# vtuber-plan/vcvits

Hardware: AMD Instinct MI355X
Metric: training utterances/sec (gen+disc step) at base.json segment_size (higher is better)
Workload: dtype f32; 1 GPU; configs/base.json widths, HiFi-GAN generator + MPD(8 periods+S) + MSD + STFT/mel-L1, G step + D step + AdamW (learning rate 0: weights held at their seeded initial values); per_gpu_batch=16, global_batch=16, segment_size=16384, parallelism=dp1, process_group_ranks=1, graph_recording_steps_before_warmup=3

## Files before the change

### include/vcvits_hip.h

```cpp
#ifndef VCVITS_HIP_H
#define VCVITS_HIP_H

#include <stdint.h>

#ifdef __cplusplus
extern "C" {
#endif

#define VCV_OK 0
#define VCV_EINVAL (-1)
#define VCV_EHIP (-2)
#define VCV_ELDS (-3)

#define VCV_ACT_NONE 0
#define VCV_ACT_LEAKY 1
#define VCV_ACT_RELU 2
#define VCV_ACT_TANH 3
#define VCV_ACT_LOGCLAMP 4

#define VCV_TF_NONE 0
#define VCV_TF_LEAKY 1
#define VCV_TF_DLEAKY 2
#define VCV_TF_DRELU 3
#define VCV_TF_DTANH 4
// ... 100 lines not shown

int vcv_conv_m1_fwd(const float* x, const float* w, const float* bias, float* y, int B, int C, int Tin,
                    int Tout, int P, int K, int stride, int dil, int pad, int in_leaky, int out_act,
                    float slope, void* stream);
int vcv_conv_c1_fwd(const float* x, const float* w, const float* bias, float* y, int B, int M, int Tin, int Tout,
                    int P, int K, int stride, int dil, int pad, int out_act, float slope, void* stream);
int vcv_conv_c1_fwd_masked(const float* x, const float* w, const float* bias, float* y, const float* oaux, int B, int M,
                           int Tin, int Tout, int P, int K, int stride, int dil, int pad, int out_act, float slope,
                           void* stream);
int vcv_conv_c1_fwd_flip(const float* x, const float* w, const float* bias, float* y, const float* oaux, int B, int M, int Tin,
                         int Tout, int P, int K, int stride, int dil, int pad, int out_act, float slope, int flip_taps,
                         void* stream);
int vcv_conv_c1_dgrad(const float* dy, const float* w, float* dx, int B, int M, int Tin, int Tout, int P, int K,
                      int stride, int dil, int pad, void* stream);
int vcv_linear_t1_fwd(const float* x, const float* w, const float* bias, float* y, int B, int C, int M, void* stream);
int vcv_linear_t1_dgrad(const float* dy, const float* w, float* dx, int B, int C, int M, void* stream);
int vcv_linear_t1_wgrad(const float* dy, const float* x, float* dw, int B, int C, int M, void* stream);
int vcv_thin_wgrad(const float* a, const float* bsh, const float* aaux, const float* baux, float* dw, int B,
                   int M, int C, int Ta, int Tb, int P, int K, int s, int d, int off, int a_tf, int b_tf,
                   float slope, float alpha, void* stream);

int vcv_grouped41_fwd(const float* x, const float* w, const float* bias, float* y, int B, int G, int Mg, int Tin,
                      int Tout, int out_act, float slope, void* stream);
int vcv_grouped41_fwd_bf16(const float* x, const float* w, const float* bias, float* y, int B, int G, int Mg, int Tin, int Tout,
                           int out_act, float slope, void* stream);
int vcv_grouped41_dgrad(const float* dy, const float* yaux, const float* w, float* dx, int B, int G, int Mg, int Tin,
                        int Tout, int dtf, float slope, void* stream);
int vcv_grouped41_dgrad_bf16(const float* dy, const float* yaux, const float* w, float* dx, int B, int G, int Mg, int Tin, int Tout,
                             int dtf, float slope, void* stream);
int vcv_grouped41_wgrad(const float* dy, const float* yaux, const float* x, float* dw, int B, int G, int Mg, int Tin,
                        int Tout, int dtf, float slope, void* stream);
int vcv_grouped41_wgrad_bf16(const float* dy, const float* yaux, const float* x, float* dw, int B, int G, int Mg, int Tin, int Tout,
                             int dtf, float slope, void* stream);

int vcv_bias_grad(const float* dy, const float* aux, float* dbias, int B, int C, int T, int tf, float slope,
                  int accumulate, void* stream);

int vcv_weight_norm_fwd(const float* v, const float* g, float* w, float* norm, int R, int C, void* stream);
int vcv_weight_norm_bwd(const float* dw, const float* v, const float* g, const float* norm, float* dv,
                        float* dg, int R, int C, void* stream);
int vcv_weight_norm_many_fwd(const void* items_dev, int n_items, int total_rows, float* wbuf, float* norm,
                             void* stream);
int vcv_weight_norm_many_bwd(const void* items_dev, int n_items, int total_rows, const float* norm, void* stream);

int vcv_spectral_norm_fwd(const float* w, float* u, float* v, float* w_sn, float* sigma, float* work, int R, int N,
                          int power_iteration, float eps, void* stream);
int vcv_spectral_norm_bwd(const float* dw_sn, const float* w_sn, const float* u, const float* v, const float* sigma,
                          float* dw, float* work, int R, int N, void* stream);

int vcv_weight_flip_transpose(const float* w, float* wt, int M, int C, int K, void* stream);

int vcv_act_grad(const float* dy, const float* y, float* out, int tf, float slope, int64_t n, void* stream);
int vcv_act_grad_add(const float* dy, const float* add, const float* y, float* out, int tf, float slope, int64_t n, void* stream);
int vcv_act_grad_bias(const float* dy, const float* y, float* out, float* dbias, int B, int C, int T, int tf, float slope,
                      void* stream);

int vcv_avg3(const float* a, const float* b, const float* c, float* y, int64_t n, void* stream);
int vcv_scale(const float* x, float* y, float alpha, int64_t n, void* stream);
int vcv_mask_mul(const float* x, const float* mask, float* y, int B, int C, int T, void* stream);
int vcv_reflect_pad_fwd(const float* x, float* y, int R, int T, int Tp, void* stream);
int vcv_reflect_pad_bwd(const float* dy, float* dx, int R, int T, int Tp, void* stream);
int vcv_avgpool4_fwd(const float* x, float* y, int R, int T, void* stream);
int vcv_avgpool4_bwd(const float* dy, float* dx, int R, int T, void* stream);

int vcv_loss_sum(const float* a, const float* b, float target, int mode, float scale, float* out,
                 int64_t n, void* stream);
// ... 186 lines not shown
```

### vcvits_amd/_lib.py

```python
import ctypes
import os

import torch

_HERE = os.path.dirname(os.path.abspath(__file__))
from . import tuning

LIB_PATH = tuning.text("VCVITS_HIP_LIB", "", "path of another build of libvcvits_hip.so (A/B builds)") or \
    os.path.join(_HERE, "csrc", "libvcvits_hip.so")

VCV_OK = 0
ACT_NONE, ACT_LEAKY, ACT_RELU, ACT_TANH, ACT_LOGCLAMP = 0, 1, 2, 3, 4
TF_NONE, TF_LEAKY, TF_DLEAKY, TF_DRELU, TF_DTANH, TF_DLOGCLAMP = 0, 1, 2, 3, 4, 5

_f32p = ctypes.c_void_p
_i32 = ctypes.c_int32


class VcvConvArgs(ctypes.Structure):
    _fields_ = [
        ("x", _f32p), ("w", _f32p), ("bias", _f32p), ("res", _f32p), ("mask", _f32p),
        ("xaux", _f32p), ("oaux", _f32p), ("y", _f32p),
        ("B", _i32), ("G", _i32), ("Cg", _i32), ("Mg", _i32),
        ("Tin", _i32), ("Tout", _i32), ("P", _i32),
# ... 39 lines not shown
_lib = None


def lib():
    global _lib
    if _lib is None:
        if not os.path.exists(LIB_PATH):
            raise RuntimeError(
                "libvcvits_hip.so not found at %s -- run `python -m vcvits_amd.build_ext` "
                "(there is no CPU fallback for the vcvits hot path)" % LIB_PATH)
        L = ctypes.CDLL(LIB_PATH)
        L.vcv_version.restype = ctypes.c_char_p
        for name in EXPORTS:
            fn = getattr(L, name)
            if name != "vcv_version":
                fn.restype = (ctypes.c_int64 if name in ("vcv_conv_dma_workspace", "vcv_wgrad_bf16_scratch", "vcv_wgrad_x3_scratch", "vcv_layernorm_c_bwd_scratch", "vcv_resblock_pair_supported",
                                                                "vcv_rel_attn_stream_bwd_workspace")
                              else ctypes.c_void_p if name == "vcv_get_seed_offset_ptr" else ctypes.c_int)
                fn.argtypes = _ARGTYPES[name]
        _lib = L
    return _lib


EXPORTS = [
    "vcv_version", "vcv_conv_gemm", "vcv_conv_wgrad", "vcv_conv_wgrad_takes_dma", "vcv_conv_wgrad_split_terms", "vcv_bias_grad",
    "vcv_weight_norm_fwd", "vcv_weight_norm_bwd", "vcv_spectral_norm_fwd", "vcv_spectral_norm_bwd", "vcv_avg3", "vcv_scale", "vcv_mask_mul",
    "vcv_reflect_pad_fwd", "vcv_reflect_pad_bwd", "vcv_avgpool4_fwd", "vcv_avgpool4_bwd",
    "vcv_loss_sum", "vcv_loss_grad", "vcv_adamw", "vcv_stft_mag_fwd", "vcv_stft_mag_bwd",
    "vcv_wn_gate_fwd", "vcv_wn_gate_bwd", "vcv_row_sum", "vcv_wn_res_skip_fwd", "vcv_wn_res_skip_bwd",
    "vcv_split_sample_fwd", "vcv_split_sample_bwd", "vcv_coupling", "vcv_layernorm_c_fwd",
    "vcv_layernorm_c_bwd", "vcv_rel_softmax_fwd", "vcv_rel_value_fwd", "vcv_rel_softmax_bwd",
    "vcv_kl_fwd", "vcv_kl_bwd", "vcv_nearest_fwd", "vcv_nearest_bwd", "vcv_nearest_raw_fwd", "vcv_nearest_raw_bwd", "vcv_slice_fwd", "vcv_slice_bwd",
    "vcv_dropout", "vcv_prof_begin", "vcv_prof_end", "vcv_prof_dump", "vcv_conv_m1_fwd", "vcv_conv_c1_fwd", "vcv_conv_c1_fwd_masked", "vcv_conv_c1_fwd_flip", "vcv_conv_c1_dgrad", "vcv_linear_t1_fwd", "vcv_linear_t1_dgrad", "vcv_linear_t1_wgrad", "vcv_thin_wgrad", "vcv_weight_flip_transpose",
    "vcv_act_grad", "vcv_act_grad_add", "vcv_weight_norm_many_fwd", "vcv_weight_norm_many_bwd", "vcv_loss_many_sum", "vcv_loss_many_grad", "vcv_conv_dma_workspace", "vcv_conv_dma", "vcv_conv_dma_plan", "vcv_conv_dma_run", "vcv_stft_complex_fwd", "vcv_istft", "vcv_grouped41_fwd", "vcv_grouped41_fwd_bf16", "vcv_grouped41_dgrad", "vcv_grouped41_dgrad_bf16", "vcv_grouped41_wgrad", "vcv_grouped41_wgrad_bf16",
    "vcv_prior_sample", "vcv_prof_bytes", "vcv_conv_bf16_plan", "vcv_conv_bf16_run", "vcv_wgrad_bf16_scratch", "vcv_wgrad_bf16", "vcv_act_grad_bias", "vcv_conv_pk_plan", "vcv_conv_pk_run",
    "vcv_conv_x3_plan", "vcv_conv_x3_run", "vcv_conv_x3_set_terms", "vcv_conv_x3_get_terms", "vcv_conv_x3_set_all", "vcv_wgrad_x3_scratch", "vcv_wgrad_x3", "vcv_rel_attn_supported", "vcv_rel_attn_fwd", "vcv_rel_attn_bwd", "vcv_rel_attn_bwd2", "vcv_set_deterministic", "vcv_get_deterministic", "vcv_prof_roof", "vcv_prof_pause", "vcv_conv_x3_pack_job", "vcv_conv_pk_pack_job", "vcv_conv_bf16_pack_job", "vcv_pack_many", "vcv_upload_table",
    "vcv_conv_bf16io_plan", "vcv_conv_bf16io_run", "vcv_cast_f32_x16", "vcv_cast_x16_f32", "vcv_conv_m1_x16_fwd",
    "vcv_prof_active", "vcv_set_seed_offset_ptr", "vcv_get_seed_offset_ptr", "vcv_pack_many_prepared", "vcv_adamw_dev", "vcv_set_words", "vcv_tuning_set", "vcv_tuning_get", "vcv_embedding_t_fwd", "vcv_embedding_t_fwd_checked", "vcv_embedding_t_bwd", "vcv_conv_x3_set_variant", "vcv_conv_plan_describe", "vcv_wgrad_bf16_set_force", "vcv_layernorm_c_bwd_scratch", "vcv_layernorm_c_bwd_ws", "vcv_resblock_pair_supported", "vcv_resblock_pair_pack", "vcv_resblock_pair_x16",
    "vcv_pyin_yin", "vcv_pyin_obs", "vcv_pyin_viterbi",
    "vcv_resample_table", "vcv_resample_apply", "vcv_phase_vocoder", "vcv_istft_ordered",
    "vcv_hubert_bias_gelu", "vcv_hubert_groupnorm_gelu", "vcv_hubert_layernorm_c_gelu", "vcv_hubert_attn_supported", "vcv_hubert_attn_fwd",
    "vcv_hubert_groupnorm_gelu_len", "vcv_hubert_mask_frames", "vcv_hubert_attn_fwd_len",
    "vcv_rel_attn_stream_supported", "vcv_rel_attn_stream_fwd",
    "vcv_rel_attn_stream_train_fwd", "vcv_rel_attn_stream_bwd_workspace", "vcv_rel_attn_stream_bwd",
    "vcv_rel_attn_stream_fwd_bf16", "vcv_hubert_attn_fwd_bf16", "vcv_hubert_attn_fwd_len_bf16",
]


_P, _I, _L, _F, _D = ctypes.c_void_p, ctypes.c_int, ctypes.c_int64, ctypes.c_float, ctypes.c_double
_ARGTYPES = {
    "vcv_conv_gemm": [ctypes.POINTER(VcvConvArgs), _P],
    "vcv_conv_wgrad": [ctypes.POINTER(VcvWgradArgs), _P],
    "vcv_conv_wgrad_takes_dma": [ctypes.POINTER(VcvWgradArgs)],
    "vcv_conv_wgrad_split_terms": [ctypes.POINTER(VcvWgradArgs)],
    "vcv_bias_grad": [_P, _P, _P, _I, _I, _I, _I, _F, _I, _P],
    "vcv_weight_norm_fwd": [_P, _P, _P, _P, _I, _I, _P],
    "vcv_weight_norm_bwd": [_P, _P, _P, _P, _P, _P, _I, _I, _P],
    "vcv_spectral_norm_fwd": [_P, _P, _P, _P, _P, _P, _I, _I, _I, _F, _P],
    "vcv_spectral_norm_bwd": [_P, _P, _P, _P, _P, _P, _P, _I, _I, _P],
    "vcv_avg3": [_P, _P, _P, _P, _L, _P],
    "vcv_scale": [_P, _P, _F, _L, _P],
    "vcv_mask_mul": [_P, _P, _P, _I, _I, _I, _P],
    "vcv_reflect_pad_fwd": [_P, _P, _I, _I, _I, _P],
    "vcv_reflect_pad_bwd": [_P, _P, _I, _I, _I, _P],
    "vcv_avgpool4_fwd": [_P, _P, _I, _I, _P],
    "vcv_avgpool4_bwd": [_P, _P, _I, _I, _P],
    "vcv_loss_sum": [_P, _P, _F, _I, _F, _P, _L, _P],
# ... 20 lines not shown
    "vcv_dropout": [_P, _P, _L, _F, ctypes.c_uint64, _P],
    "vcv_rel_value_fwd": [_P, _P, _P, _I, _I, _I, _I, _I, _P],
    "vcv_rel_softmax_bwd": [_P, _P, _P, _P, _P, _P, _P, _P, _P, _P, _P, _P, _I, _I, _I, _I, _I, _F, _P],
    "vcv_rel_attn_supported": [_I, _I, _I, _I, _I],
    "vcv_rel_attn_fwd": [_P, _P, _P, _P, _P, _P, _P, _P, _P, _I, _I, _I, _I, _I, _F, _F, ctypes.c_uint64, _I, _P],
    "vcv_rel_attn_bwd": [_P, _P, _P, _P, _P, _P, _P, _P, _P, _P, _P, _P, _P, _P, _I, _I, _I, _I, _I, _F, _F, ctypes.c_uint64, _I, _P],
    "vcv_rel_attn_bwd2": [_P, _P, _P, _P, _P, _P, _P, _P, _P, _P, _P, _P, _P, _P, _P, _I, _I, _I, _I, _I, _F, _F, ctypes.c_uint64, _I, _P],
    "vcv_set_deterministic": [_I],
    "vcv_get_deterministic": [],
    "vcv_kl_fwd": [_P, _P, _P, _P, _P, _P, _I, _I, _I, _P],
    "vcv_kl_bwd": [_P, _P, _P, _P, _P, _P, _P, _P, _P, _P, _I, _I, _I, _P],
    "vcv_nearest_fwd": [_P, _P, _I, _I, _I, _P],
    "vcv_nearest_bwd": [_P, _P, _I, _I, _I, _P],
    "vcv_nearest_raw_fwd": [_P, _P, _I, _I, _I, _P, _P],
    "vcv_nearest_raw_bwd": [_P, _P, _I, _I, _I, _P, _P],
    "vcv_slice_fwd": [_P, _P, _I, _P, _I, _I, _I, _I, _P],
    "vcv_slice_bwd": [_P, _P, _I, _P, _I, _I, _I, _I, _P],
    "vcv_conv_m1_fwd": [_P, _P, _P, _P, _I, _I, _I, _I, _I, _I, _I, _I, _I, _I, _I, _F, _P],
    "vcv_conv_c1_fwd": [_P, _P, _P, _P, _I, _I, _I, _I, _I, _I, _I, _I, _I, _I, _F, _P],
    "vcv_conv_c1_fwd_masked": [_P, _P, _P, _P, _P, _I, _I, _I, _I, _I, _I, _I, _I, _I, _I, _F, _P],
    "vcv_conv_c1_fwd_flip": [_P, _P, _P, _P, _P, _I, _I, _I, _I, _I, _I, _I, _I, _I, _I, _F, _I, _P],
    "vcv_linear_t1_fwd": [_P, _P, _P, _P, _I, _I, _I, _P],
    "vcv_linear_t1_dgrad": [_P, _P, _P, _I, _I, _I, _P],
    "vcv_linear_t1_wgrad": [_P, _P, _P, _I, _I, _I, _P],
    "vcv_conv_c1_dgrad": [_P, _P, _P, _I, _I, _I, _I, _I, _I, _I, _I, _I, _P],
    "vcv_thin_wgrad": [_P, _P, _P, _P, _P, _I, _I, _I, _I, _I, _I, _I, _I, _I, _I, _I, _I, _F, _F, _P],
    "vcv_weight_flip_transpose": [_P, _P, _I, _I, _I, _P],
    "vcv_grouped41_fwd": [_P, _P, _P, _P, _I, _I, _I, _I, _I, _I, _F, _P],
    "vcv_grouped41_fwd_bf16": [_P, _P, _P, _P, _I, _I, _I, _I, _I, _I, _F, _P],
    "vcv_grouped41_dgrad": [_P, _P, _P, _P, _I, _I, _I, _I, _I, _I, _F, _P],
    "vcv_grouped41_dgrad_bf16": [_P, _P, _P, _P, _I, _I, _I, _I, _I, _I, _F, _P],
    "vcv_grouped41_wgrad": [_P, _P, _P, _P, _I, _I, _I, _I, _I, _I, _F, _P],
    "vcv_grouped41_wgrad_bf16": [_P, _P, _P, _P, _I, _I, _I, _I, _I, _I, _F, _P],
    "vcv_act_grad": [_P, _P, _P, _I, _F, _L, _P],
    "vcv_act_grad_add": [_P, _P, _P, _P, _I, _F, _L, _P],
    "vcv_act_grad_bias": [_P, _P, _P, _P, _I, _I, _I, _I, _F, _P],
    "vcv_stft_complex_fwd": [_P, _P, _P, _P, _I, _I, _I, _I, _I, _I, _P],
    "vcv_istft": [_P, _P, _P, _P, _P, _I, _I, _I, _I, _I, _P],
    "vcv_loss_many_sum": [_P, _I, _I, _F, _I, _P, _P],
    "vcv_loss_many_grad": [_P, _I, _I, _F, _I, _P, _P, _P],
    "vcv_weight_norm_many_fwd": [_P, _I, _I, _P, _P, _P],
    "vcv_weight_norm_many_bwd": [_P, _I, _I, _P, _P],
    "vcv_conv_dma_workspace": [ctypes.POINTER(VcvConvArgs)],
    "vcv_conv_dma": [ctypes.POINTER(VcvConvArgs), _P, _I, _P],
    "vcv_conv_dma_plan": [ctypes.POINTER(VcvConvArgs), _I, ctypes.POINTER(ctypes.c_int64)],
    "vcv_conv_dma_run": [ctypes.POINTER(VcvConvArgs), _P, _P, _I, _I, _P],
    "vcv_prior_sample": [_P, _P, _P, _P, _L, _F, _P],
    "vcv_conv_bf16_plan": [ctypes.POINTER(VcvConvArgs), _I, ctypes.POINTER(ctypes.c_int64)],
    "vcv_conv_bf16_run": [ctypes.POINTER(VcvConvArgs), _P, _P, _I, _I, _P],
    "vcv_conv_pk_plan": [ctypes.POINTER(VcvConvArgs), _I, ctypes.POINTER(ctypes.c_int64)],
    "vcv_conv_pk_run": [ctypes.POINTER(VcvConvArgs), _P, _P, _I, _I, _P],
    "vcv_conv_x3_plan": [ctypes.POINTER(VcvConvArgs), _I, ctypes.POINTER(ctypes.c_int64)],
    "vcv_conv_plan_describe": [ctypes.POINTER(VcvConvArgs), _I, _I, ctypes.POINTER(ctypes.c_int32)],
    "vcv_conv_x3_run": [ctypes.POINTER(VcvConvArgs), _P, _P, _I, _I, _P],
    "vcv_conv_x3_set_terms": [_I],
    "vcv_conv_x3_get_terms": [],
    "vcv_conv_x3_set_all": [_I],
    "vcv_conv_x3_set_variant": [_I, _I, _I],
    "vcv_wgrad_bf16_set_force": [_I, _I],
    "vcv_wgrad_bf16_scratch": [ctypes.POINTER(VcvWgradArgs)],
    "vcv_wgrad_x3_scratch": [ctypes.POINTER(VcvWgradArgs)],
    "vcv_wgrad_x3": [ctypes.POINTER(VcvWgradArgs), _P, _L, _P],
    "vcv_wgrad_bf16": [ctypes.POINTER(VcvWgradArgs), _P, _L, _P],
    "vcv_prof_begin": [_I],
    "vcv_prof_end": [ctypes.POINTER(ctypes.c_double), _I],
    "vcv_prof_dump": [ctypes.c_char_p],
# ... 174 lines not shown
```

### vcvits_amd/csrc/conv_grouped.hip

```cpp
#include "common.h"

namespace {

constexpr int CG = 4, K = 41, S = 4, PAD = 20, KP = 44;

template <int N, int LB, class Src, class Dst>
__device__ __forceinline__ void stage_n(int tid, Src src, Dst dst) {
  constexpr int IT = (N + 255) / 256;
#pragma unroll
  for (int i0 = 0; i0 < IT; i0 += LB) {
    float v[LB];
#pragma unroll
    for (int l = 0; l < LB; ++l) {
      const int i = tid + (i0 + l) * 256;
      v[l] = (i0 + l < IT && i < N) ? src(i) : 0.f;
    }
#pragma unroll
    for (int l = 0; l < LB; ++l) {
      const int i = tid + (i0 + l) * 256;
      if (i0 + l < IT && i < N) dst(i, v[l]);
    }
  }
}

template <int N, int LB, class Src, class Aux, class Dst>
__device__ __forceinline__ void stage_n2(int tid, bool want_aux, Src src, Aux aux, Dst dst) {
  constexpr int IT = (N + 255) / 256;
#pragma unroll
  for (int i0 = 0; i0 < IT; i0 += LB) {
    float v[LB], a[LB];
#pragma unroll
    for (int l = 0; l < LB; ++l) {
      const int i = tid + (i0 + l) * 256;
// ... 306 lines not shown
    const int k = 4 * tg + kq;
    float v[4];
#pragma unroll
    for (int ci = 0; ci < 4; ++ci) v[ci] = k < K ? wg[((size_t)m * CG + ci) * K + k] : 0.f;
    wsb[tg][kq][m] = pack_bf16x4(v[0], v[1], v[2], v[3]);
  }
  __syncthreads();
  const int n = lane & 15, kq = lane >> 4;
  f32x4_t acc[4];
#pragma unroll
  for (int tl = 0; tl < 4; ++tl) acc[tl] = (f32x4_t){0.f, 0.f, 0.f, 0.f};
  const int tw = wave * 64;
#pragma unroll
  for (int tg = 0; tg < NTG; ++tg) {
    const s16x4_t a = wsb[tg][kq][n];
#pragma unroll
    for (int tl = 0; tl < 4; ++tl)
      acc[tl] = __builtin_amdgcn_mfma_f32_16x16x16bf16_1k(a, xs[kq][tw + tl * 16 + n + tg], acc[tl], 0, 0, 0);
  }
#pragma unroll
  for (int tl = 0; tl < 4; ++tl) {
    const int t = t0 + tw + tl * 16 + n;
    if (t >= Tout) continue;
#pragma unroll
    for (int r = 0; r < 4; ++r) {
      const int m = kq * 4 + r;
      float v = acc[tl][r] + (bias ? bias[g * MG + m] : 0.f);
      y[((size_t)b * G * MG + (size_t)g * MG + m) * Tout + t] = vcv_act(v, act, slope);
    }
  }
}
}

extern "C" int vcv_grouped41_fwd_bf16(const float* x, const float* w, const float* bias, float* y, int B, int G, int Mg,
                                      int Tin, int Tout, int out_act, float slope, void* stream) {
  if (!x || !w || !y || B <= 0 || G <= 0 || Tin <= 0 || Tout <= 0 || Mg != 16) return VCV_EINVAL;
  hipLaunchKernelGGL(grouped_fwd_mfma_bf16_kernel, dim3(vcv_cdiv(Tout, 256), G, B), dim3(256), 0, (hipStream_t)stream, x, w, bias,
                     y, G, Tin, Tout, out_act, slope);
  return vcv_check_launch();
}

extern "C" int vcv_grouped41_fwd(const float* x, const float* w, const float* bias, float* y, int B, int G, int Mg,
                                 int Tin, int Tout, int out_act, float slope, void* stream) {
  if (!x || !w || !y || B <= 0 || G <= 0 || Tin <= 0 || Tout <= 0 || (Mg != 4 && Mg != 16)) return VCV_EINVAL;
  dim3 grid(vcv_cdiv(Tout, 256), G, B);
  if (Mg == 16) hipLaunchKernelGGL(grouped_fwd_mfma_kernel, grid, dim3(256), 0, (hipStream_t)stream, x, w, bias, y, G, Tin, Tout, out_act, slope);
  else if (Tout <= 64)
    hipLaunchKernelGGL((grouped_fwd_kernel<4, 64>), dim3(vcv_cdiv(Tout, 64), vcv_cdiv(G, 4), B), dim3(256), 0, (hipStream_t)stream, x,
                       w, bias, y, G, Tin, Tout, out_act, slope);
  else if (Tout <= 128)
    hipLaunchKernelGGL((grouped_fwd_kernel<4, 128>), dim3(vcv_cdiv(Tout, 128), vcv_cdiv(G, 2), B), dim3(256), 0, (hipStream_t)stream,
                       x, w, bias, y, G, Tin, Tout, out_act, slope);
  else
    hipLaunchKernelGGL((grouped_fwd_kernel<4, 256>), grid, dim3(256), 0, (hipStream_t)stream, x, w, bias, y, G, Tin, Tout, out_act,
                       slope);
  return vcv_check_launch();
}

namespace {
__global__ void __launch_bounds__(256)
grouped_dgrad_mfma_kernel(const float* __restrict__ dy, const float* __restrict__ yaux, const float* __restrict__ w,
                          float* __restrict__ dx, int G, int Tin, int Tout, int dtf, float slope) {
  constexpr int MG = 16, QT = 256, NJ = 11;
  constexpr int DSP = 272;
  __shared__ float ds[MG][DSP];
  __shared__ float wsd[NJ * 4][64];
  const int tid = threadIdx.x, lane = tid & 63, wave = tid >> 6;
  const int q0 = blockIdx.x * QT, g = blockIdx.y, b = blockIdx.z;
  const size_t ybase = ((size_t)b * G * MG + (size_t)g * MG) * Tout;
  {
    auto at = [&](int i, bool& ok) {
      const int m = i / DSP, t = q0 - 5 + i - m * DSP;
      ok = t >= 0 && t < Tout;
      return ybase + (size_t)m * Tout + t;
    };
    stage_n2<MG * DSP, 9>(tid, dtf == VCV_TF_DLEAKY,
        [&](int i) { bool ok; const size_t gi = at(i, ok); return ok ? dy[gi] : 0.f; },
        [&](int i) { bool ok; const size_t gi = at(i, ok); return ok ? yaux[gi] : 1.f; },
        [&](int i, float v, float a) { (&ds[0][0])[i] = v * vcv_dleaky(a, slope); });
// ... 96 lines not shown
  }
  float* dxr = dx + ((size_t)b * G * CG + (size_t)g * CG + kq) * Tin;
#pragma unroll
  for (int tl = 0; tl < 4; ++tl) {
    const int q = q0 + qw + tl * 16 + n;
    const int u = 4 * q;
    if (u + 3 < Tin && (Tin & 3) == 0) {
      *reinterpret_cast<f32x4_t*>(dxr + u) = acc[tl];
    } else {
#pragma unroll
      for (int r = 0; r < 4; ++r)
        if (u + r < Tin) dxr[u + r] = acc[tl][r];
    }
  }
}
}

extern "C" int vcv_grouped41_dgrad_bf16(const float* dy, const float* yaux, const float* w, float* dx, int B, int G, int Mg,
                                        int Tin, int Tout, int dtf, float slope, void* stream) {
  if (!dy || !w || !dx || B <= 0 || G <= 0 || Tin <= 0 || Tout <= 0 || Mg != 16) return VCV_EINVAL;
  if (dtf != VCV_TF_NONE && dtf != VCV_TF_DLEAKY) return VCV_EINVAL;
  if (dtf >= VCV_TF_DLEAKY && !yaux) return VCV_EINVAL;
  hipLaunchKernelGGL(grouped_dgrad_mfma_bf16_kernel, dim3(vcv_cdiv(vcv_cdiv(Tin, 4), 256), G, B), dim3(256), 0, (hipStream_t)stream, dy,
                     yaux, w, dx, G, Tin, Tout, dtf, slope);
  return vcv_check_launch();
}

extern "C" int vcv_grouped41_dgrad(const float* dy, const float* yaux, const float* w, float* dx, int B, int G, int Mg,
                                   int Tin, int Tout, int dtf, float slope, void* stream) {
  if (!dy || !w || !dx || B <= 0 || G <= 0 || Tin <= 0 || Tout <= 0 || (Mg != 4 && Mg != 16)) return VCV_EINVAL;
  if (dtf != VCV_TF_NONE && dtf != VCV_TF_DLEAKY) return VCV_EINVAL;
  if (dtf >= VCV_TF_DLEAKY && !yaux) return VCV_EINVAL;
  dim3 grid(vcv_cdiv(vcv_cdiv(Tin, 4), 256), G, B);
  if (Mg == 16) hipLaunchKernelGGL(grouped_dgrad_mfma_kernel, grid, dim3(256), 0, (hipStream_t)stream, dy, yaux, w, dx, G, Tin, Tout, dtf, slope);
  else {
    const int nq = vcv_cdiv(Tin, 4);
    if (nq <= 64)
      hipLaunchKernelGGL((grouped_dgrad_kernel<4, 64>), dim3(vcv_cdiv(nq, 64), vcv_cdiv(G, 4), B), dim3(256), 0, (hipStream_t)stream, dy,
                         yaux, w, dx, G, Tin, Tout, dtf, slope);
    else if (nq <= 128)
      hipLaunchKernelGGL((grouped_dgrad_kernel<4, 128>), dim3(vcv_cdiv(nq, 128), vcv_cdiv(G, 2), B), dim3(256), 0, (hipStream_t)stream,
                         dy, yaux, w, dx, G, Tin, Tout, dtf, slope);
    else
      hipLaunchKernelGGL((grouped_dgrad_kernel<4, 256>), grid, dim3(256), 0, (hipStream_t)stream, dy, yaux, w, dx, G, Tin, Tout, dtf,
                         slope);
  }
  return vcv_check_launch();
}

namespace {
template <bool BF>
__global__ void __launch_bounds__(256)
grouped_wgrad_mfma_kernel(const float* __restrict__ dy, const float* __restrict__ yaux, const float* __restrict__ x,
                          float* __restrict__ dw, int G, int Tin, int Tout, int dtf, float slope, int nstage, int uper,
                          int nunit) {
  constexpr int MG = 16, TT = 256, NT = 11, NW = CG * K;
  constexpr int SPAN = S * TT + KP, DP = TT + 1;
  __shared__ float xs[CG][SPAN];
  __shared__ float ds[MG][DP];
  __shared__ float racc[MG][NT * 16];
  const int tid = threadIdx.x, lane = tid & 63, wave = tid >> 6;
  const int g = blockIdx.x;
  const int u_lo = blockIdx.y * uper, u_hi = u_lo + uper < nunit ? u_lo + uper : nunit;
  const int j16 = lane & 15, kk = lane >> 4;
  int boff[NT];
#pragma unroll
  for (int nt = 0; nt < NT; ++nt) {
// ... 118 lines not shown
```

### vcvits_amd/csrc/tuning.h

```cpp
#pragma once

struct VcvTuning {
  int xcd_remap = 1;
  int pk_ws = 1;
  int pk_ws_bf16 = 0;
  int pk_x4 = 1;
  int pk_vec = 1;
  int x3_variant = -1;
  int x3_v6 = 1;
  int x3_js2 = 1;
  int x3_merge_phases = 1;
  int x3_old_ks = 0;
  int x3_all = 0;
  int x3_terms = 6;
  int wgrad_dma = 1;
  int wgrad_tile = -1;
  int wgrad_verbose = 0;
  int wgrad_dma_split = 1;
  int wgrad_bf16_ws = 1;
  int wgrad_finish_vec = 1;
  int bias_rows = 1;
  int c1_chunk = 0;
  int m1_lds = 1;
  int c1_wgrad_pairs = 1;
  int thin_wgrad_wgs = 2048;
  int act_grad_vec = 1;
  int ln_regs = 1;
  int stft_wave = 1;
  int attn_rows = 1;
  int zero_memset = 0;
  int pack_tile = 1;
  int pack_tile_bf16 = 1;
  int pair_dbg = 0;
  int pair_grid = 0;
  int pair_stream = 1;
  int deterministic = 0;
};

VcvTuning& vcv_tuning();
extern "C" int vcv_tuning_set(const char* key, int value);
extern "C" int vcv_tuning_get(const char* key, int* value);
```

### vcvits_amd/csrc/version.hip

```cpp
#include "common.h"
#include <cstring>
extern "C" const char* vcv_version(void) {
  return "vcvits_hip gfx950 fp32-mfma(32x32x2) conv family; built " __DATE__ " " __TIME__;
}

extern "C" int vcv_set_deterministic(int on) {
  vcv_tuning().deterministic = on ? 1 : 0;
  return VCV_OK;
}
extern "C" int vcv_get_deterministic(void) { return vcv_tuning().deterministic; }

namespace {
struct TuningKey { const char* name; int VcvTuning::*field; };
#define TK(f) {#f, &VcvTuning::f}
const TuningKey kTuningKeys[] = {
    TK(xcd_remap), TK(pk_ws), TK(pk_ws_bf16), TK(pk_x4), TK(pk_vec), TK(x3_variant), TK(x3_v6), TK(x3_js2), TK(x3_merge_phases), TK(x3_old_ks), TK(x3_all),
    TK(x3_terms), TK(wgrad_dma), TK(wgrad_tile), TK(wgrad_verbose), TK(wgrad_dma_split), TK(wgrad_bf16_ws), TK(wgrad_finish_vec), TK(bias_rows),
    TK(c1_chunk), TK(m1_lds), TK(c1_wgrad_pairs), TK(thin_wgrad_wgs), TK(act_grad_vec), TK(ln_regs), TK(stft_wave), TK(attn_rows),
    TK(zero_memset), TK(pack_tile), TK(pack_tile_bf16), TK(pair_dbg), TK(pair_grid), TK(pair_stream), TK(deterministic)};
#undef TK
int VcvTuning::*find_key(const char* key, size_t len) {
  for (const TuningKey& k : kTuningKeys)
    if (strlen(k.name) == len && strncmp(k.name, key, len) == 0) return k.field;
  return nullptr;
}
VcvTuning make_tuning() {
  VcvTuning t;
  const char* det = getenv("VCVITS_DETERMINISTIC");
  if (det && det[0] == '1') t.deterministic = 1;
  const char* e = getenv("VCVITS_TUNING");
  while (e && *e) {
    const char* end = strchr(e, ',');
    const size_t n = end ? (size_t)(end - e) : strlen(e);
    const char* eq = (const char*)memchr(e, '=', n);
    if (eq) {
      int VcvTuning::*f = find_key(e, (size_t)(eq - e));
      if (f) t.*f = atoi(eq + 1);
      else fprintf(stderr, "vcvits_hip: VCVITS_TUNING: unknown key '%.*s'\n", (int)(eq - e), e);
    } else if (n) {
      fprintf(stderr, "vcvits_hip: VCVITS_TUNING: '%.*s' is not key=value\n", (int)n, e);
    }
    e = end ? end + 1 : nullptr;
  }
  if (t.x3_terms != 9) t.x3_terms = 6;
  return t;
}
}
VcvTuning& vcv_tuning() {
  static VcvTuning t = make_tuning();
  return t;
}
extern "C" int vcv_tuning_set(const char* key, int value) {
// ... 19 lines not shown
```

### vcvits_amd/tuning.py

```python
import os

REGISTRY = {}


def _declare(name, kind, default, doc, value):
    REGISTRY[name] = (kind, default, doc, value)
    return value


def flag(name, default, doc):
    raw = os.environ.get(name)
    return _declare(name, "flag", default, doc, default if raw is None else raw == "1")


def integer(name, default, doc):
    raw = os.environ.get(name)
    return _declare(name, "int", default, doc, default if raw is None else int(raw))


def number(name, default, doc):
    raw = os.environ.get(name)
    return _declare(name, "float", default, doc, default if raw is None else float(raw))


def text(name, default, doc):
    return _declare(name, "text", default, doc, os.environ.get(name, default))


def live_flag(name):
    kind, default, doc, _ = REGISTRY[name]
    raw = os.environ.get(name)
    return default if raw is None else (raw == "1" if kind == "flag" else int(raw))


KERNEL_KEYS = ("xcd_remap", "pk_ws", "pk_ws_bf16", "pk_x4", "pk_vec", "x3_variant", "x3_v6", "x3_js2", "x3_merge_phases", "x3_old_ks", "x3_all", "x3_terms",
               "wgrad_dma", "wgrad_tile", "wgrad_verbose", "wgrad_dma_split", "wgrad_bf16_ws", "wgrad_finish_vec", "bias_rows", "c1_chunk", "m1_lds",
               "c1_wgrad_pairs", "thin_wgrad_wgs", "act_grad_vec", "ln_regs", "stft_wave", "attn_rows", "zero_memset", "pack_tile",
               "pack_tile_bf16", "pair_dbg", "pair_grid", "pair_stream", "deterministic")


def kernel_get(key):
    import ctypes
    from ._lib import check, lib
    v = ctypes.c_int(0)
    check(lib().vcv_tuning_get(key.encode(), ctypes.byref(v)), "vcv_tuning_get(%s)" % key)
    return v.value


def kernel_set(key, value):
    from ._lib import check, lib
    check(lib().vcv_tuning_set(key.encode(), int(value)), "vcv_tuning_set(%s)" % key)


def table():
    import importlib
    for mod in ("vcvits_amd._lib", "vcvits_amd.ops", "vcvits_amd.mel_processing", "vcvits_amd.model.flow", "vcvits_amd.model.modules",
                "vcvits_amd.model.discriminators._pair", "vcvits_amd.light.optim", "vcvits_amd.light.graphed"):
        importlib.import_module(mod)
    out = ["environment variables of the host side (name, default, meaning):"]
    for name in sorted(REGISTRY):
        kind, default, doc, value = REGISTRY[name]
        d = ("1" if default else "0") if kind == "flag" else str(default)
        out.append("  %-28s %-10s %s" % (name, d, doc))
    out.append("")
    out.append("kernel tuning table (VCVITS_TUNING=\"key=value,...\"; csrc/tuning.h documents each key):")
    try:
        out.append("  " + ", ".join("%s=%d" % (k, kernel_get(k)) for k in KERNEL_KEYS))
    except Exception as e:
        out.append("  (library not loaded: %s)" % e)
    return out

# ... 5 lines not shown
```

Measured before the change: 255.1 utterances/s.

## Add persistent wave-level grouped conv fwd/dgrad kernels with double-buffered LDS prefetch

Adds persistent kernels for the grouped (Mg=16, 41-tap MSD-style) conv forward and data-gradient. Each wave walks a contiguous run of (group, batch, tile) items and holds the group's weights in registers across items. It double-buffers the input tile in per-wave LDS, overlapping the global loads for the next tile with the MFMA loop of the current one. The grid is sized from an occupancy query and capped at two blocks per CU. This replaces one short-lived workgroup per 256-sample tile, cutting launch/tail overhead and redundant weight loads, at the cost of per-wave load imbalance and higher register/LDS pressure.

```diff
diff --git a/include/vcvits_hip.h b/include/vcvits_hip.h
--- a/include/vcvits_hip.h
+++ b/include/vcvits_hip.h
@@ -156,6 +156,7 @@
                         int Tout, int dtf, float slope, void* stream);
 int vcv_grouped41_wgrad_bf16(const float* dy, const float* yaux, const float* x, float* dw, int B, int G, int Mg, int Tin, int Tout,
                              int dtf, float slope, void* stream);
+int vcv_grouped41_form(int which, int B, int G, int Mg, int Tin, int Tout, int* out);
 
 int vcv_bias_grad(const float* dy, const float* aux, float* dbias, int B, int C, int T, int tf, float slope,
                   int accumulate, void* stream);
diff --git a/vcvits_amd/_lib.py b/vcvits_amd/_lib.py
--- a/vcvits_amd/_lib.py
+++ b/vcvits_amd/_lib.py
@@ -95,7 +95,7 @@
     "vcv_layernorm_c_bwd", "vcv_rel_softmax_fwd", "vcv_rel_value_fwd", "vcv_rel_softmax_bwd",
     "vcv_kl_fwd", "vcv_kl_bwd", "vcv_nearest_fwd", "vcv_nearest_bwd", "vcv_nearest_raw_fwd", "vcv_nearest_raw_bwd", "vcv_slice_fwd", "vcv_slice_bwd",
     "vcv_dropout", "vcv_prof_begin", "vcv_prof_end", "vcv_prof_dump", "vcv_conv_m1_fwd", "vcv_conv_c1_fwd", "vcv_conv_c1_fwd_masked", "vcv_conv_c1_fwd_flip", "vcv_conv_c1_dgrad", "vcv_linear_t1_fwd", "vcv_linear_t1_dgrad", "vcv_linear_t1_wgrad", "vcv_thin_wgrad", "vcv_weight_flip_transpose",
-    "vcv_act_grad", "vcv_act_grad_add", "vcv_weight_norm_many_fwd", "vcv_weight_norm_many_bwd", "vcv_loss_many_sum", "vcv_loss_many_grad", "vcv_conv_dma_workspace", "vcv_conv_dma", "vcv_conv_dma_plan", "vcv_conv_dma_run", "vcv_stft_complex_fwd", "vcv_istft", "vcv_grouped41_fwd", "vcv_grouped41_fwd_bf16", "vcv_grouped41_dgrad", "vcv_grouped41_dgrad_bf16", "vcv_grouped41_wgrad", "vcv_grouped41_wgrad_bf16",
+    "vcv_act_grad", "vcv_act_grad_add", "vcv_weight_norm_many_fwd", "vcv_weight_norm_many_bwd", "vcv_loss_many_sum", "vcv_loss_many_grad", "vcv_conv_dma_workspace", "vcv_conv_dma", "vcv_conv_dma_plan", "vcv_conv_dma_run", "vcv_stft_complex_fwd", "vcv_istft", "vcv_grouped41_fwd", "vcv_grouped41_fwd_bf16", "vcv_grouped41_dgrad", "vcv_grouped41_dgrad_bf16", "vcv_grouped41_wgrad", "vcv_grouped41_wgrad_bf16", "vcv_grouped41_form",
     "vcv_prior_sample", "vcv_prof_bytes", "vcv_conv_bf16_plan", "vcv_conv_bf16_run", "vcv_wgrad_bf16_scratch", "vcv_wgrad_bf16", "vcv_act_grad_bias", "vcv_conv_pk_plan", "vcv_conv_pk_run",
     "vcv_conv_x3_plan", "vcv_conv_x3_run", "vcv_conv_x3_set_terms", "vcv_conv_x3_get_terms", "vcv_conv_x3_set_all", "vcv_wgrad_x3_scratch", "vcv_wgrad_x3", "vcv_rel_attn_supported", "vcv_rel_attn_fwd", "vcv_rel_attn_bwd", "vcv_rel_attn_bwd2", "vcv_set_deterministic", "vcv_get_deterministic", "vcv_prof_roof", "vcv_prof_pause", "vcv_conv_x3_pack_job", "vcv_conv_pk_pack_job", "vcv_conv_bf16_pack_job", "vcv_pack_many", "vcv_upload_table",
     "vcv_conv_bf16io_plan", "vcv_conv_bf16io_run", "vcv_cast_f32_x16", "vcv_cast_x16_f32", "vcv_conv_m1_x16_fwd",
@@ -182,6 +182,7 @@
     "vcv_grouped41_dgrad_bf16": [_P, _P, _P, _P, _I, _I, _I, _I, _I, _I, _F, _P],
     "vcv_grouped41_wgrad": [_P, _P, _P, _P, _I, _I, _I, _I, _I, _I, _F, _P],
     "vcv_grouped41_wgrad_bf16": [_P, _P, _P, _P, _I, _I, _I, _I, _I, _I, _F, _P],
+    "vcv_grouped41_form": [_I, _I, _I, _I, _I, _I, ctypes.POINTER(ctypes.c_int)],
     "vcv_act_grad": [_P, _P, _P, _I, _F, _L, _P],
     "vcv_act_grad_add": [_P, _P, _P, _P, _I, _F, _L, _P],
     "vcv_act_grad_bias": [_P, _P, _P, _P, _I, _I, _I, _I, _F, _P],
diff --git a/vcvits_amd/csrc/conv_grouped.hip b/vcvits_amd/csrc/conv_grouped.hip
--- a/vcvits_amd/csrc/conv_grouped.hip
+++ b/vcvits_amd/csrc/conv_grouped.hip
@@ -1,4 +1,5 @@
 #include "common.h"
+#include <type_traits>
 
 namespace {
 
@@ -371,6 +372,364 @@
 }
 }
 
+namespace {
+constexpr int P_NW = 4;
+constexpr int P_TT = 64;
+constexpr int P_WPC = 2;
+struct G41Part { int nitem, ntile, grid, nrun, base, rem; };
+
+__device__ __forceinline__ void wave_lds_fence() {
+  __builtin_amdgcn_fence(__ATOMIC_RELEASE, "wavefront");
+  __builtin_amdgcn_wave_barrier();
+  __builtin_amdgcn_fence(__ATOMIC_ACQUIRE, "wavefront");
+}
+
+template <class T = float>
+__device__ __forceinline__ T* at_bytes(T* base, unsigned byte_off) {
+  typedef typename std::conditional<std::is_const<T>::value, const char, char>::type C;
+  return reinterpret_cast<T*>(reinterpret_cast<C*>(base) + byte_off);
+}
+
+__device__ __forceinline__ int lane_here(int lane) {
+  asm volatile("" : "+v"(lane));
+  return lane;
+}
+
+__device__ __forceinline__ void g41_run(const G41Part& p, int run, int& lo, int& hi) {
+  lo = run * p.base + (run < p.rem ? run : p.rem);
+  hi = lo + p.base + (run < p.rem ? 1 : 0);
+}
+
+constexpr int PF_QN = P_TT + 10;
+constexpr int PF_QP = 76;
+constexpr int PF_BUF = CG * 4 * PF_QP;
+constexpr int PF_OP = 68;
+constexpr int PF_LD = (4 * PF_QN + 63) / 64;
+constexpr int PF_H = 3, PF_K1 = 24;
+
+__global__ void __launch_bounds__(256, 4)
+grouped_fwd_persist_kernel(const float* __restrict__ x, const float* __restrict__ w, const float* __restrict__ bias,
+                           float* __restrict__ y, int B, int G, int Tin, int Tout, int leaky, float slope, int vec, G41Part p) {
+  constexpr int MG = 16;
+  __shared__ __attribute__((aligned(16))) float lds[P_NW][2][PF_BUF];
+  const int lane0 = threadIdx.x & 63;
+  const int wave = __builtin_amdgcn_readfirstlane(threadIdx.x >> 6);
+  int it, hi;
+  g41_run(p, blockIdx.x * P_NW + wave, it, hi);
+  if (it >= hi) return;
+  const int n0 = lane0 & 15, kq0 = lane0 >> 4;
+  int tile = __builtin_amdgcn_readfirstlane(it % p.ntile), b = __builtin_amdgcn_readfirstlane((it / p.ntile) % B),
+      g = __builtin_amdgcn_readfirstlane(it / p.ntile / B);
+  float* const buf = &lds[wave][0][0];
+  auto load_span = [&](float (&v)[CG][PF_H], int g_, int b_, int tile_, int h) {
+    const float* xb = x + ((size_t)b_ * G * CG + (size_t)g_ * CG) * Tin;
+    const int in0 = tile_ * P_TT * S - PAD;
+    const int lane = lane_here(lane0);
+#pragma unroll
+    for (int u = 0; u < PF_H; ++u) {
+      const int l = h * PF_H + u, j = lane + 64 * l, ti = in0 + j;
+      if (l < PF_LD) {
+        const unsigned o = (j < 4 * PF_QN && ti >= 0 && ti < Tin) ? 4 * ti : 0;
+#pragma unroll
+        for (int ci = 0; ci < CG; ++ci) v[ci][u] = *at_bytes(xb + (size_t)ci * Tin, o);
+      }
+    }
+  };
+  auto store_span = [&](const float (&v)[CG][PF_H], float* xs, int tile_, int h) {
+    const int in0 = tile_ * P_TT * S - PAD;
+    const int lane = lane_here(lane0);
+    const int wofs = (lane & 3) * PF_QP + (lane >> 2);
+#pragma unroll
+    for (int u = 0; u < PF_H; ++u) {
+      const int l = h * PF_H + u, j = lane + 64 * l, ti = in0 + j;
+      const bool ok = ti >= 0 && ti < Tin;
+      if (l < PF_LD && j < 4 * PF_QN) {
+#pragma unroll
+        for (int ci = 0; ci < CG; ++ci) xs[ci * 4 * PF_QP + wofs + 16 * l] = ok ? v[ci][u] : 0.f;
+      }
+    }
+  };
+  float a[K], bv[4];
+  auto load_weights = [&](int g_) {
+    const float* wg = w + (size_t)g_ * MG * CG * K;
+    const int lane = lane_here(lane0), n = lane & 15, kq = lane >> 4;
+    const unsigned wo = (n * CG + kq) * K * 4;
+#pragma unroll
+    for (int k = 0; k < K; ++k) a[k] = *at_bytes(wg + k, wo);
+#pragma unroll
+    for (int r = 0; r < 4; ++r) bv[r] = bias ? bias[g_ * MG + kq * 4 + r] : 0.f;
+#pragma unroll
+    for (int k = 0; k < K; ++k) asm volatile("" ::"v"(a[k]));
+  };
+  float v[CG][PF_H];
+  {
+    float v1[CG][PF_H];
+    load_span(v, g, b, tile, 0);
+    load_span(v1, g, b, tile, 1);
+    load_weights(g);
+    store_span(v, buf, tile, 0);
+    store_span(v1, buf, tile, 1);
+  }
+  int gw = g, cur = 0;
+  for (;;) {
+    if (g != gw) load_weights(g), gw = g;
+    int ntile = tile + 1, nb = b, ng = g;
+    if (ntile == p.ntile) {
+      ntile = 0;
+      if (++nb == B) nb = 0, ++ng;
+    }
+    const bool more = it + 1 < hi;
+    if (more) load_span(v, ng, nb, ntile, 0);
+    wave_lds_fence();
+    float* const xs = buf + cur * PF_BUF;
+    const float* xr = xs + kq0 * 4 * PF_QP + n0;
+    f32x4_t acc[4];
+#pragma unroll
+    for (int tl = 0; tl < 4; ++tl) acc[tl] = (f32x4_t){0.f, 0.f, 0.f, 0.f};
+#pragma unroll
+    for (int k = 0; k < K; ++k) {
+      if (k == PF_K1 && more) {
+        __builtin_amdgcn_sched_barrier(0);
+        store_span(v, buf + (cur ^ 1) * PF_BUF, ntile, 0);
+        load_span(v, ng, nb, ntile, 1);
+      }
+#pragma unroll
+      for (int tl = 0; tl < 4; ++tl)
+        acc[tl] = __builtin_amdgcn_mfma_f32_16x16x4f32(a[k], xr[(k & 3) * PF_QP + (k >> 2) + tl * 16], acc[tl], 0, 0, 0);
+    }
+    wave_lds_fence();
+    const int lane = lane_here(lane0), n = lane & 15, kq = lane >> 4;
+#pragma unroll
+    for (int tl = 0; tl < 4; ++tl)
+#pragma unroll
+      for (int r = 0; r < 4; ++r) {
+        const float t = acc[tl][r] + bv[r];
+        xs[(kq * 4 + r) * PF_OP + tl * 16 + n] = leaky ? vcv_leaky(t, slope) : t;
+      }
+    wave_lds_fence();
+    const int t0 = tile * P_TT;
+    float* yb = y + ((size_t)b * G * MG + (size_t)g * MG) * Tout + t0;
+    if (vec && t0 + P_TT <= Tout) {
+#pragma unroll
+      for (int i = 0; i < 4; ++i) {
+        const int row = i * 4 + kq, c4 = n * 4;
+        *reinterpret_cast<f32x4_t*>(at_bytes(yb + (size_t)(i * 4) * Tout, 4u * (kq * Tout + c4))) =
+            *reinterpret_cast<const f32x4_t*>(xs + row * PF_OP + c4);
+      }
+    } else if (t0 + lane < Tout) {
+#pragma unroll
+      for (int row = 0; row < MG; ++row) *at_bytes(yb + (size_t)row * Tout, 4u * lane) = xs[row * PF_OP + lane];
+    }
+    if (!more) break;
+    __builtin_amdgcn_sched_barrier(0);
+    store_span(v, buf + (cur ^ 1) * PF_BUF, ntile, 1);
+    cur ^= 1, ++it, tile = ntile, b = nb, g = ng;
+  }
+}
+
+constexpr int PD_COLS = P_TT + 10;
+constexpr int PD_DSP = 80;
+constexpr int PD_BUF = 16 * PD_DSP;
+constexpr int PD_N = 16 * PD_COLS;
+constexpr int PD_LD = (PD_N + 63) / 64;
+constexpr int PD_NC = 3, PD_H = (PD_LD + PD_NC - 1) / PD_NC;
+
+__global__ void __launch_bounds__(256, 4)
+grouped_dgrad_persist_kernel(const float* __restrict__ dy, const float* __restrict__ yaux, const float* __restrict__ w,
+                             float* __restrict__ dx, int B, int G, int Tin, int Tout, int dtf, float slope, G41Part p) {
+  constexpr int MG = 16, NJ = 11;
+  __shared__ float lds[P_NW][2][PD_BUF];
+  const int lane0 = threadIdx.x & 63;
+  const int wave = __builtin_amdgcn_readfirstlane(threadIdx.x >> 6);
+  int it, hi;
+  g41_run(p, blockIdx.x * P_NW + wave, it, hi);
+  if (it >= hi) return;
+  const int n0 = lane0 & 15, kq0 = lane0 >> 4;
+  int tile = __builtin_amdgcn_readfirstlane(it % p.ntile), b = __builtin_amdgcn_readfirstlane((it / p.ntile) % B),
+      g = __builtin_amdgcn_readfirstlane(it / p.ntile / B);
+  float* const buf = &lds[wave][0][0];
+  const bool want_aux = dtf == VCV_TF_DLEAKY;
+  auto slot = [&](int lane, int L, int& m, int& c) {
+    if (L < 16) {
+      m = L, c = lane;
+      return true;
+    }
+    const int e = lane + 64 * (L - 16);
+    m = e / 10, c = 64 + e - m * 10;
+    return L < PD_LD && e < 16 * 10;
+  };
+  auto load_rows = [&](float (&v)[PD_H], float (&ax)[PD_H], int g_, int b_, int tile_, int h) {
+    const size_t ybase = ((size_t)b_ * G * MG + (size_t)g_ * MG) * Tout;
+    const int q0 = tile_ * P_TT;
+    const int lane = lane_here(lane0);
+    unsigned o[PD_H];
+#pragma unroll
+    for (int u = 0; u < PD_H; ++u) {
+      const int L = h * PD_H + u;
+      int m, c;
+      const bool in = slot(lane, L, m, c);
+      const int t = q0 - 5 + c;
+      const bool ok = in && t >= 0 && t < Tout;
+      o[u] = ok ? 4 * (L < 16 ? t : m * Tout + t) : 0;
+      v[u] = *at_bytes(dy + ybase + (L < 16 ? (size_t)L * Tout : 0), o[u]);
+    }
+    const float* au = want_aux ? yaux : dy;
+#pragma unroll
+    for (int u = 0; u < PD_H; ++u) {
+      const int L = h * PD_H + u;
+      ax[u] = *at_bytes(au + ybase + (L < 16 ? (size_t)L * Tout : 0), o[u]);
+    }
+  };
+  auto store_rows = [&](const float (&v)[PD_H], const float (&ax)[PD_H], float* ds, int tile_, int h) {
+    const int q0 = tile_ * P_TT;
+    const int lane = lane_here(lane0);
+#pragma unroll
+    for (int u = 0; u < PD_H; ++u) {
+      int m, c;
+      if (slot(lane, h * PD_H + u, m, c)) {
+        const int t = q0 - 5 + c;
+        const bool ok = t >= 0 && t < Tout;
+        ds[m * PD_DSP + c] = (ok ? v[u] : 0.f) * vcv_dleaky((ok && want_aux) ? ax[u] : 1.f, slope);
+      }
+    }
+  };
+  float a[NJ * 4];
+  auto load_weights = [&](int g_) {
+    const int lane = lane_here(lane0), kq = lane >> 4, ci = (lane >> 2) & 3, r = lane & 3;
+    const float* wg = w + (size_t)g_ * MG * CG * K;
+    const unsigned wo = ((kq * CG + ci) * K + r) * 4;
+#pragma unroll
+    for (int j = 0; j < NJ; ++j)
+#pragma unroll
+      for (int mc = 0; mc < 4; ++mc) {
+        const float t = *at_bytes(wg + mc * 4 * CG * K, wo + (4 * j + r < K ? 16 * j : 0));
+        a[j * 4 + mc] = 4 * j + r < K ? t : 0.f;
+      }
+#pragma unroll
+    for (int i = 0; i < NJ * 4; ++i) asm volatile("" ::"v"(a[i]));
+  };
+  float v[PD_H], ax[PD_H];
+  {
+    static_assert(PD_NC == 3, "the first item's parts are written out one by one");
+    float v1[PD_H], ax1[PD_H], v2[PD_H], ax2[PD_H];
+    load_rows(v, ax, g, b, tile, 0);
+    load_rows(v1, ax1, g, b, tile, 1);
+    load_rows(v2, ax2, g, b, tile, 2);
+    load_weights(g);
+    store_rows(v, ax, buf, tile, 0);
+    store_rows(v1, ax1, buf, tile, 1);
+    store_rows(v2, ax2, buf, tile, 2);
+  }
+  int gw = g, cur = 0;
+  for (;;) {
+    if (g != gw) load_weights(g), gw = g;
+    int ntile = tile + 1, nb = b, ng = g;
+    if (ntile == p.ntile) {
+      ntile = 0;
+      if (++nb == B) nb = 0, ++ng;
+    }
+    const bool more = it + 1 < hi;
+    if (more) load_rows(v, ax, ng, nb, ntile, 0);
+    wave_lds_fence();
+    const float* dr = buf + cur * PD_BUF + kq0 * PD_DSP + n0 + 10;
+    f32x4_t acc[4];
+#pragma unroll
+    for (int tl = 0; tl < 4; ++tl) acc[tl] = (f32x4_t){0.f, 0.f, 0.f, 0.f};
+#pragma unroll
+    for (int j = 0; j < NJ; ++j) {
+#pragma unroll
+      for (int c = 1; c < PD_NC; ++c)
+        if (j == (c * NJ + PD_NC - 1) / PD_NC && more) {
+          __builtin_amdgcn_sched_barrier(0);
+          store_rows(v, ax, buf + (cur ^ 1) * PD_BUF, ntile, c - 1);
+          load_rows(v, ax, ng, nb, ntile, c);
+        }
+#pragma unroll
+      for (int mc = 0; mc < 4; ++mc)
+#pragma unroll
+        for (int tl = 0; tl < 4; ++tl)
+          acc[tl] = __builtin_amdgcn_mfma_f32_16x16x4f32(a[j * 4 + mc], dr[mc * 4 * PD_DSP - j + tl * 16], acc[tl], 0, 0, 0);
+    }
+    float* dxg = dx + ((size_t)b * G * CG + (size_t)g * CG) * Tin;
+    const int lane = lane_here(lane0), n = lane & 15, kq = lane >> 4;
+#pragma unroll
+    for (int tl = 0; tl < 4; ++tl) {
+      const int u = 4 * (tile * P_TT + tl * 16 + n);
+      const unsigned o = 4u * (kq * Tin + u);
+      if (u + 3 < Tin && (Tin & 3) == 0) {
+        *reinterpret_cast<f32x4_t*>(at_bytes(dxg, o)) = acc[tl];
+      } else {
+#pragma unroll
+        for (int r = 0; r < 4; ++r)
+          if (u + r < Tin) *at_bytes(dxg + r, o) = acc[tl][r];
+      }
+    }
+    if (!more) break;
+    __builtin_amdgcn_sched_barrier(0);
+    store_rows(v, ax, buf + (cur ^ 1) * PD_BUF, ntile, PD_NC - 1);
+    cur ^= 1, ++it, tile = ntile, b = nb, g = ng;
+  }
+}
+
+int g41_slots(int which) {
+  static int cache[2] = {0, 0};
+  if (cache[which] > 0) return cache[which];
+  int dev = 0, cus = 0, per = 0;
+  hipError_t e = hipGetDevice(&dev);
+  if (e == hipSuccess) e = hipDeviceGetAttribute(&cus, hipDeviceAttributeMultiprocessorCount, dev);
+  if (e == hipSuccess)
+    e = which == 0 ? hipOccupancyMaxActiveBlocksPerMultiprocessor(&per, grouped_fwd_persist_kernel, 64 * P_NW, 0)
+                   : hipOccupancyMaxActiveBlocksPerMultiprocessor(&per, grouped_dgrad_persist_kernel, 64 * P_NW, 0);
+  if (e != hipSuccess || cus <= 0 || per <= 0) {
+    (void)hipGetLastError();
+    return 256 * P_WPC;
+  }
+  return cache[which] = cus * (per < P_WPC ? per : P_WPC);
+}
+
+bool g41_persist_plan(int which, int B, int G, int Mg, int Tin, int Tout, G41Part& p) {
+  if (Mg != 16 || !vcv_tuning().grouped41_persist) return false;
+  const int ntile = vcv_cdiv(which == 0 ? Tout : vcv_cdiv(Tin, 4), P_TT);
+  if (which == 1) {
+    const int nq = vcv_cdiv(Tin, 4);
+    if (4ll * nq >= 3ll * 256 * vcv_cdiv(nq, 256)) return false;
+  }
+  const long long nitem = (long long)G * B * ntile;
+  if (nitem >= (1ll << 31) || Tin >= (1 << 26) || Tout >= (1 << 26)) return false;
+  const int forced = vcv_tuning().grouped41_grid;
+  const long long cap = forced > 0 ? forced : g41_slots(which), need = (nitem + P_NW - 1) / P_NW;
+  p.nitem = (int)nitem, p.ntile = ntile;
+  p.grid = (int)(need < cap ? need : cap);
+  const int nwave = p.grid * P_NW;
+  p.base = p.nitem / nwave, p.rem = p.nitem % nwave;
+  p.nrun = p.nitem < nwave ? p.nitem : nwave;
+  return true;
+}
+}
+
+extern "C" int vcv_grouped41_form(int which, int B, int G, int Mg, int Tin, int Tout, int* out) {
+  if (!out || which < 0 || which > 2 || B <= 0 || G <= 0 || Tin <= 0 || Tout <= 0 || (Mg != 4 && Mg != 16)) return VCV_EINVAL;
+  G41Part p;
+  if (which < 2 && g41_persist_plan(which, B, G, Mg, Tin, Tout, p)) {
+    out[0] = 1, out[1] = p.nitem, out[2] = p.nrun, out[3] = p.grid;
+    return VCV_OK;
+  }
+  long long wgs;
+  if (which == 2 && Mg == 16) {
+    const int nunit = B * vcv_cdiv(Tout, 256);
+    int per_group = 512 / G < 1 ? 1 : 512 / G;
+    if (per_group > nunit) per_group = nunit;
+    if (vcv_get_deterministic()) per_group = 1;
+    wgs = (long long)G * vcv_cdiv(nunit, vcv_cdiv(nunit, per_group));
+  } else if (Mg == 16) {
+    wgs = (long long)vcv_cdiv(which == 0 ? Tout : vcv_cdiv(Tin, 4), 256) * G * B;
+  } else {
+    wgs = 0;
+  }
+  out[0] = 0, out[1] = out[2] = out[3] = (int)wgs;
+  return VCV_OK;
+}
+
 extern "C" int vcv_grouped41_fwd_bf16(const float* x, const float* w, const float* bias, float* y, int B, int G, int Mg,
                                       int Tin, int Tout, int out_act, float slope, void* stream) {
   if (!x || !w || !y || B <= 0 || G <= 0 || Tin <= 0 || Tout <= 0 || Mg != 16) return VCV_EINVAL;
@@ -383,7 +742,11 @@
                                  int Tin, int Tout, int out_act, float slope, void* stream) {
   if (!x || !w || !y || B <= 0 || G <= 0 || Tin <= 0 || Tout <= 0 || (Mg != 4 && Mg != 16)) return VCV_EINVAL;
   dim3 grid(vcv_cdiv(Tout, 256), G, B);
-  if (Mg == 16) hipLaunchKernelGGL(grouped_fwd_mfma_kernel, grid, dim3(256), 0, (hipStream_t)stream, x, w, bias, y, G, Tin, Tout, out_act, slope);
+  G41Part part;
+  if ((out_act == VCV_ACT_NONE || out_act == VCV_ACT_LEAKY) && g41_persist_plan(0, B, G, Mg, Tin, Tout, part))
+    hipLaunchKernelGGL(grouped_fwd_persist_kernel, dim3(part.grid), dim3(64 * P_NW), 0, (hipStream_t)stream, x, w, bias, y, B, G, Tin,
+                       Tout, (int)(out_act == VCV_ACT_LEAKY), slope, (int)((Tout & 3) == 0 && ((uintptr_t)y & 15) == 0), part);
+  else if (Mg == 16) hipLaunchKernelGGL(grouped_fwd_mfma_kernel, grid, dim3(256), 0, (hipStream_t)stream, x, w, bias, y, G, Tin, Tout, out_act, slope);
   else if (Tout <= 64)
     hipLaunchKernelGGL((grouped_fwd_kernel<4, 64>), dim3(vcv_cdiv(Tout, 64), vcv_cdiv(G, 4), B), dim3(256), 0, (hipStream_t)stream, x,
                        w, bias, y, G, Tin, Tout, out_act, slope);
@@ -546,7 +909,11 @@
   if (dtf != VCV_TF_NONE && dtf != VCV_TF_DLEAKY) return VCV_EINVAL;
   if (dtf >= VCV_TF_DLEAKY && !yaux) return VCV_EINVAL;
   dim3 grid(vcv_cdiv(vcv_cdiv(Tin, 4), 256), G, B);
-  if (Mg == 16) hipLaunchKernelGGL(grouped_dgrad_mfma_kernel, grid, dim3(256), 0, (hipStream_t)stream, dy, yaux, w, dx, G, Tin, Tout, dtf, slope);
+  G41Part part;
+  if (g41_persist_plan(1, B, G, Mg, Tin, Tout, part))
+    hipLaunchKernelGGL(grouped_dgrad_persist_kernel, dim3(part.grid), dim3(64 * P_NW), 0, (hipStream_t)stream, dy, yaux, w, dx, B, G,
+                       Tin, Tout, dtf, slope, part);
+  else if (Mg == 16) hipLaunchKernelGGL(grouped_dgrad_mfma_kernel, grid, dim3(256), 0, (hipStream_t)stream, dy, yaux, w, dx, G, Tin, Tout, dtf, slope);
   else {
     const int nq = vcv_cdiv(Tin, 4);
     if (nq <= 64)
diff --git a/vcvits_amd/csrc/tuning.h b/vcvits_amd/csrc/tuning.h
--- a/vcvits_amd/csrc/tuning.h
+++ b/vcvits_amd/csrc/tuning.h
@@ -29,6 +29,8 @@
   int stft_wave = 1;
   int attn_rows = 1;
   int zero_memset = 0;
+  int grouped41_persist = 1;
+  int grouped41_grid = 0;
   int pack_tile = 1;
   int pack_tile_bf16 = 1;
   int pair_dbg = 0;
diff --git a/vcvits_amd/csrc/version.hip b/vcvits_amd/csrc/version.hip
--- a/vcvits_amd/csrc/version.hip
+++ b/vcvits_amd/csrc/version.hip
@@ -17,7 +17,8 @@
     TK(xcd_remap), TK(pk_ws), TK(pk_ws_bf16), TK(pk_x4), TK(pk_vec), TK(x3_variant), TK(x3_v6), TK(x3_js2), TK(x3_merge_phases), TK(x3_old_ks), TK(x3_all),
     TK(x3_terms), TK(wgrad_dma), TK(wgrad_tile), TK(wgrad_verbose), TK(wgrad_dma_split), TK(wgrad_bf16_ws), TK(wgrad_finish_vec), TK(bias_rows),
     TK(c1_chunk), TK(m1_lds), TK(c1_wgrad_pairs), TK(thin_wgrad_wgs), TK(act_grad_vec), TK(ln_regs), TK(stft_wave), TK(attn_rows),
-    TK(zero_memset), TK(pack_tile), TK(pack_tile_bf16), TK(pair_dbg), TK(pair_grid), TK(pair_stream), TK(deterministic)};
+    TK(zero_memset), TK(pack_tile), TK(pack_tile_bf16), TK(pair_dbg), TK(pair_grid), TK(pair_stream), TK(grouped41_persist),
+    TK(grouped41_grid), TK(deterministic)};
 #undef TK
 int VcvTuning::*find_key(const char* key, size_t len) {
   for (const TuningKey& k : kTuningKeys)
diff --git a/vcvits_amd/tuning.py b/vcvits_amd/tuning.py
--- a/vcvits_amd/tuning.py
+++ b/vcvits_amd/tuning.py
@@ -36,7 +36,7 @@
 KERNEL_KEYS = ("xcd_remap", "pk_ws", "pk_ws_bf16", "pk_x4", "pk_vec", "x3_variant", "x3_v6", "x3_js2", "x3_merge_phases", "x3_old_ks", "x3_all", "x3_terms",
                "wgrad_dma", "wgrad_tile", "wgrad_verbose", "wgrad_dma_split", "wgrad_bf16_ws", "wgrad_finish_vec", "bias_rows", "c1_chunk", "m1_lds",
                "c1_wgrad_pairs", "thin_wgrad_wgs", "act_grad_vec", "ln_regs", "stft_wave", "attn_rows", "zero_memset", "pack_tile",
-               "pack_tile_bf16", "pair_dbg", "pair_grid", "pair_stream", "deterministic")
+               "pack_tile_bf16", "pair_dbg", "pair_grid", "pair_stream", "grouped41_persist", "grouped41_grid", "deterministic")
 
 
 def kernel_get(key):
```

Result: no change. 256.8 utterances/s, median of 6 (+0.7%).
